# 10XGenomics/supernova

Measured on AMD Instinct MI355X. Metric: Gk-mers/s through count+graph at k=48, 1.2B×150bp; bit-exact counts, higher is better.
Workload: dtype u64

## Files before the change

### include/snk.h

```cpp
#ifndef SNK_H_
#define SNK_H_
#include <stddef.h>
#include <stdint.h>

#ifdef __cplusplus
extern "C" {
#endif

#define SNK_OK 0
#define SNK_E_ARG (-1)
#define SNK_E_HIP (-2)
#define SNK_E_NOGPU (-3)
#define SNK_E_NOMEM (-4)
#define SNK_E_IO (-5)
#define SNK_E_UNSUPPORTED (-6)
#define SNK_E_INTERNAL (-7)

typedef struct snk_ctx snk_ctx;

typedef struct snk_params {
    uint32_t K;
    uint32_t min_qual;
    uint32_t min_freq;
    uint32_t min_bc;
// ... 26 lines not shown
    uint32_t count_tight_slots;
    uint32_t count_screen_ratio_pct;
    uint32_t target_inst;
    uint32_t bucket_fill_pct;
    uint32_t adaptive_buckets;
    uint32_t chunk_kmers;
    uint32_t minimiser_len;
    uint32_t partition_passes;
    uint32_t hot_buckets;
    uint32_t hot_min, hot_factor, hot_class_inst;
    uint32_t exchange_ranges;
    uint32_t join_ranking;
    uint32_t path_lookup;
    uint32_t unitig_bc_cut;
    uint32_t hbv_dev_min, hbv_big;
    uint32_t reserved[9];
    uint32_t last_count_kernel, last_count_limit, last_partition_passes, last_minimiser_len;
} snk_tuning;
void snk_tuning_default(snk_tuning* t);
int snk_ctx_set_tuning(snk_ctx* ctx, const snk_tuning* t, char* err, size_t errcap);
void snk_ctx_get_tuning(const snk_ctx* ctx, snk_tuning* t);
int snk_ctx_set_option(snk_ctx* ctx, const char* name, long long value, char* err, size_t errcap);
int snk_option_check(const char* name, long long value, char* err, size_t errcap);
int snk_ctx_clear_option(snk_ctx* ctx, const char* name);
int snk_ctx_get_option(const snk_ctx* ctx, const char* name, long long* value);
const char* snk_option_name(uint32_t i);
const char* snk_option_doc(uint32_t i);

typedef struct snk_synth_params {
    uint64_t seed;
    uint64_t n_reads;
// ... 398 lines not shown
```

### supernova_amd/csrc/snk_api.hip

```cpp
#include <math.h>
#include <stdlib.h>
#include <execinfo.h>
#include <dlfcn.h>
#include <time.h>

#include <algorithm>

#include "snk_ctx.h"
#include "snk_kernels.h"
#include "snk_synth.h"

static thread_local char g_last_error[512] = "";

hipError_t snk_enter(snk_ctx* ctx) { return hipSetDevice(ctx->device); }

void snk_set_mlen(snk_ctx* ctx, const snk_params* p) {
    uint32_t m = (p->flags & SNK_F_LONG_MINIMISER) ? (uint32_t)SNK_M_LONG : (uint32_t)SNK_M_OF(p->K);
    const unsigned long long v = snk_opt_u64(ctx, SNK_OPT_minimiser_len);
    if (v == SNK_M_LONG || v == SNK_M_OF(p->K)) m = (uint32_t)v;
    ctx->mlen = m;
}

void snk_set_error(char* err, size_t errcap, const char* fmt, ...) {
    va_list ap;
// ... 390 lines not shown
    }
    ctx->blocks.swap(keep);
}

extern "C" void snk_ctx_destroy(snk_ctx* ctx) {
    if (!ctx) return;
    (void)snk_enter(ctx);
    snk_ctx_release_scratch(ctx);
    snk_ctx_trim_cache(ctx);
    if (ctx->va_base) { va_unmap_from(ctx, 0); (void)hipMemAddressFree(ctx->va_base, ctx->va_size); ctx->va_base = nullptr; }
    if (ctx->shard) snk_shard_state_free(ctx->shard);
    if (ctx->host_io && ctx->host_io_free) ctx->host_io_free(ctx->host_io);
    if (ctx->df_io && ctx->df_io_free) ctx->df_io_free(ctx->df_io);
    if (ctx->shard_host && ctx->shard_host_free) ctx->shard_host_free(ctx->shard_host);
    if (ctx->stream_job && ctx->stream_job_free) ctx->stream_job_free(ctx->stream_job);
    if (ctx->stream) (void)hipStreamDestroy(ctx->stream);
    delete ctx;
}

extern "C" void snk_synth_default(snk_synth_params* sp, uint64_t n_reads, uint64_t seed, int error_free) {
    memset(sp, 0, sizeof *sp);
    sp->seed = seed;
    sp->n_reads = n_reads;
    sp->read_len = 150;
    sp->genome_len = n_reads * 150 / 56;
    if (sp->genome_len < 1000) sp->genome_len = 1000;
    sp->mol_len = 50000;
    sp->mols_per_bc = 10;
    sp->pairs_per_bc = 400;
    sp->insert_min = 300;
// ... 53 lines not shown
```

### supernova_amd/csrc/snk_ctx.h

```cpp
#pragma once
#include <hip/hip_runtime.h>
#include <stdarg.h>
#include <stdio.h>
#include <string.h>

#include <string>
#include <vector>

#include "../../include/snk.h"
#include "snk_launch.h"
#include "snk_opts.h"

struct snk_ctx {
    int device = 0;
    hipStream_t stream = nullptr;
    hipStream_t cur_stream = nullptr;
    int n_cu = 256;
    size_t lds_per_block = 65536;
    uint64_t device_mem_total = 0;
    double pass_sigma = 0.0;
    uint64_t plan_mapped = 0;
    uint64_t plan_mem = 0;
    struct block { void* p; size_t bytes; bool used; uint64_t serial = 0; uint64_t epoch = 0; };
    uint64_t call_epoch = 0;
    uint64_t alloc_serial = 0;
    std::vector<block> blocks;
    struct vrange { size_t off, bytes; };
    char* va_base = nullptr;
    size_t va_size = 0, va_mapped = 0, va_high = 0, va_high_prev[2] = {0, 0};
    std::vector<hipMemGenericAllocationHandle_t> va_handles;
    std::vector<size_t> va_chunk;
    std::vector<vrange> va_free;
    std::vector<vrange> va_used;
    size_t va_floor = 0;
    int va_state = 0;
    bool va_sealed = false;
    struct vser { size_t off; uint64_t serial; };
    std::vector<vser> va_serial;
    bool arena_legacy = false;
    size_t total_alloc = 0;
    size_t peak_alloc = 0;
    size_t cached_bytes = 0;
    uint64_t last_n_kmers = 0, last_n_instances = 0;
    uint64_t last_region_max = 0, last_region_n = 0;
    uint64_t last_bnd = 0, last_bnd_n = 0;
    uint32_t last_ovf = 0, last_ovf_nb = 0;
    uint64_t last_ovf_reads = 0;
    uint64_t last_dense = 0;
    double retain_ratio = 0.0;
    uint32_t count_screen = 0;
    uint32_t count_tight = 0;
    double screen_ratio = 0.0;
    double claim_ratio = 0.0;
    uint64_t claim_ratio_reads = 0;
    uint32_t claim_ratio_k = 0;
    uint32_t mlen = 16;
    uint32_t last_extra = 0;
    uint64_t last_input_fp = 0;
    bool have_input_fp = false;
    uint32_t last_count_limit = 0;
// ... 40 lines not shown
```

### supernova_amd/csrc/snk_local.hip

```cpp
#include <string.h>
#include <cstring>
#include <rocprim/rocprim.hpp>

#include <type_traits>

#include "snk_ctx.h"
#include "snk_common.h"
#include "snk_kernels.h"
#include "snk_graph.h"
#include "snk_stages.h"

namespace {

constexpr uint32_t NONE = 0xFFFFFFFFu;
constexpr unsigned long long NONE64 = ~0ull;
constexpr uint16_t NONE16 = 0xFFFFu;
constexpr int TB = 256;

struct chunk_src {
    const uint32_t* chunk_n;
    const uint32_t* chunk_base;
    const uint4* extra;
    const unsigned long long* region_off;
    uint32_t NB, n_extra, n_regions;
// ... 21 lines not shown
    if (r >= G) return;
    uint32_t head = NONE, total = 0, m = 0, expect = 0;
    for (uint32_t b = r; b < NB; b += G) {
        const uint32_t n = chunk_n[b];
        span[b] = 1;
        merged[b] = n;
        if (n == 0) { head = NONE; continue; }
        const uint32_t base = chunk_base[b];
        if (head != NONE && base == expect && total + n <= cap && m < 255u) {
            total += n; ++m;
            merged[head] = total; merged[b] = 0; span[head] = (uint8_t)m;
        } else { head = b; total = n; m = 1; }
        expect = base + n;
    }
}
__global__ void __launch_bounds__(256) bl_chunk_desc_kernel(chunk_src cs, uint32_t nchunks, uint4* __restrict__ desc, uint64_t region_cap, uint64_t* __restrict__ desc_src) {
    const uint32_t c = blockIdx.x * 256 + threadIdx.x;
    if (c >= nchunks) return;
    uint32_t bucket, n, off = 0, meta = 0, region;
    if (c < cs.NB) {
        bucket = c; n = cs.chunk_n[c];
        if (n) off = cs.chunk_base[c];
        region = bucket % cs.n_regions;
        if (cs.span && n && cs.span[c] > 1) meta = 0x80000000u | cs.span[c];
    } else {
        const uint4 e = cs.extra[c - cs.NB];
        bucket = e.x; off = e.y; n = e.z & 0xFFFu; region = e.z >> 12; meta = e.w;
    }
    const uint64_t base = cs.region_off[region] + off;
    desc[c] = make_uint4((uint32_t)base, n, bucket, meta);
    if (desc_src) desc_src[c] = (uint64_t)region * region_cap + off;
}
__device__ __forceinline__ chunk_t chunk_get(const uint4* __restrict__ desc, uint32_t c) {
    const uint4 d = desc[c];
    chunk_t k;
    k.base = d.x; k.n = d.y; k.bucket = d.z; k.lg = d.w >> 24; k.id = d.w & 0xFFFFFFu; k.span = 1;
    if (d.w >> 31) { k.lg = 0; k.id = 0; k.span = d.w & 0xFFFFu; }
    return k;
}

__device__ __forceinline__ snk_kmer load_key(const snk_u128* keys, uint64_t i) {
    const uint64_t* p = reinterpret_cast<const uint64_t*>(keys + i);
    snk_kmer k;
    k.lo = p[0];
    k.hi = p[1];
    return k;
// ... 2 lines not shown
    uint32_t x = (uint32_t)(hi >> 32) * 0x9E3779B1u ^ (uint32_t)hi * 0x85EBCA77u ^ (uint32_t)(lo >> 32) * 0xC2B2AE3Du ^
                 (uint32_t)lo * 0x27D4EB2Fu;
    return snk_mix32(x);
}
template <int K>
__device__ __forceinline__ uint32_t oriented_base(snk_kmer k, bool rc, int idx) {
    return rc ? (snk_kmer_base<K>(k, K - 1 - idx) ^ 3u) : snk_kmer_base<K>(k, idx);
}

template <int K, int CAP, int T, bool BIG, bool GR, int MM>
__device__ __forceinline__ void bl_prune_chunk(const uint32_t c, const uint4* __restrict__ desc, uint32_t NB, bl_shard sh, const bl_regions& rg,
                                                     const snk_u128* __restrict__ keys, const uint64_t* __restrict__ vals,
                                                     uint32_t do_prune, uint8_t* __restrict__ ctx_out,
                                                     uint32_t* __restrict__ count_out, uint8_t* __restrict__ pend_out,
                                                     uint32_t* __restrict__ nbr_out, uint32_t* __restrict__ nbnd,
                                                     uint32_t* __restrict__ biglist, uint32_t* __restrict__ nbig,
                                                     unsigned long long* __restrict__ gindex, uint64_t gmask) {
    constexpr int HT = CAP <= 256 ? 512 : 4096;
    typedef typename std::conditional<(K <= 48 && !GR), uint32_t, uint64_t>::type klo_w;
    constexpr int KLS = (K <= 48 && !GR) ? 32 : 0;
    __shared__ uint64_t khi[CAP];
    __shared__ klo_w klo[CAP];
    __shared__ uint32_t ht[HT];
    __shared__ uint32_t bcnt;
    const int tid = threadIdx.x;
    const chunk_t ch = chunk_get(desc, c);
    if (ch.n == 0) return;
    if (!BIG && ch.n > (uint32_t)CAP) {
        if (tid == 0) biglist[atomicAdd(nbig, 1u)] = c;
        return;
    }
    const uint32_t n = ch.n;
    uint64_t src = ch.base;
    if (rg.keys_r) { src = rg.desc_src[c]; keys = rg.keys_r; vals = rg.vals_r; }
    __syncthreads();
    for (int s = tid; s < HT; s += T) ht[s] = 0;
    if (tid == 0) bcnt = 0;
    constexpr int NPT = (CAP + T - 1) / T;
    uint64_t myv[NPT];
    snk_kmer kq[NPT];
#pragma unroll
    for (int q = 0; q < NPT; ++q) {
        const uint32_t i = tid + q * T;
        myv[q] = 0;
        if (i < n) {
            kq[q] = load_key(keys, src + i);
// ... 156 lines not shown
                    if (!placed) gindex[gmask + 1] = 1ull;
                }
            }
        }
    }
    snk_wave_add(&bcnt, mybnd);
    __syncthreads();
    if (tid == 0) nbnd[c] = bcnt;
}
template <int K, int CAP, int T, bool BIG, bool GR, int MM>
__global__ void __launch_bounds__(T) bl_prune_kernel(const uint4* __restrict__ desc, uint32_t NB, bl_shard sh, bl_regions rg, const uint32_t* __restrict__ biglist_in,
                                                     uint32_t nchunks, uint32_t cpw,
                                                     const snk_u128* __restrict__ keys, const uint64_t* __restrict__ vals,
                                                     uint32_t do_prune, uint8_t* __restrict__ ctx_out,
                                                     uint32_t* __restrict__ count_out, uint8_t* __restrict__ pend_out,
                                                     uint32_t* __restrict__ nbr_out, uint32_t* __restrict__ nbnd,
                                                     uint32_t* __restrict__ biglist, uint32_t* __restrict__ nbig, const uint32_t* __restrict__ n_dev,
                                                     unsigned long long* __restrict__ gindex, uint64_t gmask) {
    if (BIG && n_dev) {
        const uint32_t nb = *n_dev;
        for (uint32_t w = blockIdx.x; w < nb; w += gridDim.x)
            bl_prune_chunk<K, CAP, T, BIG, GR, MM>(biglist_in[w], desc, NB, sh, rg, keys, vals, do_prune, ctx_out, count_out, pend_out, nbr_out, nbnd, biglist, nbig, gindex, gmask);
        return;
    }
    for (uint32_t r = 0; r < cpw; ++r) {
        const uint32_t w = blockIdx.x * cpw + r;
        if (w >= nchunks) return;
        bl_prune_chunk<K, CAP, T, BIG, GR, MM>(BIG ? biglist_in[w] : w, desc, NB, sh, rg, keys, vals, do_prune, ctx_out, count_out, pend_out, nbr_out,
                                       nbnd, biglist, nbig, gindex, gmask);
    }
}

__global__ void __launch_bounds__(TB) bl_index_build_kernel(const snk_u128* __restrict__ keys, const uint8_t* __restrict__ pend,
                                                            uint64_t n, unsigned long long* __restrict__ tab, uint64_t mask) {
    const uint64_t i = (uint64_t)blockIdx.x * TB + threadIdx.x;
    if (i >= n || !pend[i]) return;
    const snk_kmer k = load_key(keys, i);
    uint32_t h1, h2;
    snk_kmer_hash2(k, &h1, &h2);
    uint64_t slot = (((uint64_t)h1 << 32) | h2) & mask;
    const unsigned long long ent = ((unsigned long long)h1 << 32) | (unsigned long long)(i + 1);
    for (;;) {
        const unsigned long long old = atomicCAS(&tab[slot], 0ull, ent);
        if (old == 0ull) break;
// ... 378 lines not shown
template <typename T>
static int excl_scan(snk_ctx* ctx, hipStream_t st, const T* in, T* out, size_t count, char* err, size_t errcap) {
    size_t tb = 0;
    SNK_HIP_TRY(rocprim::exclusive_scan((void*)nullptr, tb, in, out, (T)0, count, rocprim::plus<T>(), st));
    void* tmp;
    int rc = snk_ctx_alloc(ctx, tb, &tmp, err, errcap);
    if (rc) return rc;
    SNK_HIP_TRY(rocprim::exclusive_scan(tmp, tb, in, out, (T)0, count, rocprim::plus<T>(), st));
    return SNK_OK;
}

constexpr int SCAP = 256, ST = 64;
constexpr int BCAP = SNK_GRAPH_CHUNK_MAX, BT = 256;

namespace {
constexpr int QWORDS = 4;
constexpr int QSPAN = 8 * QWORDS * TB;
template <int K, bool FILL>
__global__ void __launch_bounds__(TB) bl_query_kernel(const snk_u128* __restrict__ keys, const uint8_t* __restrict__ premote, uint64_t n,
                                                      uint32_t NB_total, uint32_t NBl, uint32_t world, uint32_t mlen,
                                                      unsigned long long* __restrict__ qcount_or_cursor,
                                                      unsigned long long* __restrict__ qbuf) {
    extern __shared__ unsigned long long dynq[];
    __shared__ uint16_t list[QSPAN];
    __shared__ uint32_t cnt;
    uint32_t* lcur = reinterpret_cast<uint32_t*>(dynq + world);
    const uint64_t base = (uint64_t)blockIdx.x * QSPAN;
    if (threadIdx.x == 0) cnt = 0;
    for (uint32_t r = threadIdx.x; r < world; r += TB) { dynq[r] = 0; lcur[r] = 0; }
    __syncthreads();
// ... 64 lines not shown
    const uint32_t merge_cap = snk_opt_is_set(ctx, SNK_OPT_chunk_merge) ? std::min<uint32_t>(snk_opt_u32(ctx, SNK_OPT_chunk_merge), (uint32_t)SCAP) : (uint32_t)SCAP;
    if (merge_cap && tab->chunk_n && tab->NB > tab->n_regions) {
        uint8_t* span;
        uint32_t* merged;
        G_ALLOC(span, uint8_t, (uint64_t)tab->NB + 1);
        G_ALLOC(merged, uint32_t, (uint64_t)tab->NB + 1);
        SNK_HIP_TRY(snk_launch(bl_chunk_merge_kernel, snk_blocks(tab->n_regions, 256), 256, 0, st, tab->chunk_n, tab->chunk_base, tab->NB, tab->n_regions, merge_cap, span, merged));
        cs.span = span;
        cs.chunk_n = merged;
    }
    const uint32_t nchunks = tab->NB + tab->n_extra;
    B->nchunks = nchunks;
    G_ALLOC(B->desc, uint4, (uint64_t)nchunks + 1);
    uint64_t* desc_src = nullptr;
    if (tab->keys_r) G_ALLOC(desc_src, uint64_t, (uint64_t)nchunks + 1);
    SNK_HIP_TRY(snk_launch(bl_chunk_desc_kernel, snk_blocks(nchunks, 256), 256, 0, st, cs, nchunks, B->desc, tab->region_cap, desc_src));
    uint32_t *nbnd, *ctr;
    G_ALLOC(B->ctx, uint8_t, n + 16);
    G_ALLOC(B->pend, uint8_t, n + 16);
    G_ALLOC(B->counts, uint32_t, n + 4);
    G_ALLOC(B->nbr, uint32_t, n + 2);
    G_ALLOC(B->rq, uint32_t, 2 * n + 2);
    G_ALLOC(nbnd, uint32_t, (uint64_t)nchunks + 1);
    G_ALLOC(B->biglist, uint32_t, n / SCAP + 2);
    G_ALLOC(ctr, uint32_t, 16);
    B->premote = nullptr;
    if (B->world > 1 || B->force_dist) {
        G_ALLOC(B->premote, uint8_t, n + 16);
        SNK_HIP_TRY(hipMemsetAsync(B->premote, 0, n + 16, st));
    }
    SNK_HIP_TRY(hipMemsetAsync(nbnd, 0, ((uint64_t)nchunks + 1) * 4, st));
    SNK_HIP_TRY(hipMemsetAsync(ctr, 0, 64, st));
    bl_shard sh;
    sh.bucket_base = B->premote ? B->rank * B->NBl : 0u;
    sh.NBl = B->premote ? B->NBl : 0u;
    sh.me = B->rank;
    sh.G = tab->n_regions ? tab->n_regions : 1u;
    sh.premote = B->premote;
    const uint32_t NBh = B->premote ? B->NB_total : tab->NB;
    const uint32_t cpw = snk_opt_u32(ctx, SNK_OPT_bl_cpw);
    uint64_t tg0 = 0;
    unsigned long long* index0 = nullptr;
    if (snk_opt_u32(ctx, SNK_OPT_bl_index_fused)) {
        const uint64_t guess = (ctx->last_bnd_n == n && ctx->last_bnd) ? ctx->last_bnd + ctx->last_bnd / 8 : n / 5;
        tg0 = 1024;
        while (tg0 < 2 * guess) tg0 <<= 1;
        G_ALLOC(index0, unsigned long long, tg0 + 1);
        SNK_HIP_TRY(hipMemsetAsync(index0, 0, (tg0 + 1) * 8, st));
    }
    bl_regions rg;
    rg.keys_r = tab->keys_r; rg.vals_r = tab->vals_r; rg.desc_src = desc_src;
    rg.keys_dense = const_cast<snk_u128*>(tab->keys);
    const bool long_m = ctx->mlen == (uint32_t)SNK_M_LONG;
    SNK_HIP_TRY(snk_launch(long_m ? bl_prune_kernel<K, SCAP, ST, false, GR, SNK_M_LONG> : bl_prune_kernel<K, SCAP, ST, false, GR, SNK_M_OF(K)>, snk_blocks(nchunks, cpw), ST, 0, st, (const uint4*)B->desc, NBh, sh, rg,
                           (const uint32_t*)nullptr, nchunks, cpw, tab->keys, tab->vals, B->do_prune | (snk_opt_u32(ctx, SNK_OPT_bl_noclassify) ? 2u : 0u), B->ctx, B->counts, B->pend, B->nbr, nbnd,
                           B->biglist, ctr, (const uint32_t*)nullptr, index0, tg0 - 1));
    uint32_t h_nbig = 0;
    SNK_HIP_TRY(hipMemcpyAsync(ctr + 1, ctr, 4, hipMemcpyDeviceToDevice, st));
    SNK_HIP_TRY(snk_launch(long_m ? bl_prune_kernel<K, BCAP, BT, true, GR, SNK_M_LONG> : bl_prune_kernel<K, BCAP, BT, true, GR, SNK_M_OF(K)>, 2048, BT, 0, st, (const uint4*)B->desc, NBh, sh, rg,
                           (const uint32_t*)B->biglist, 0u, 1u, tab->keys, tab->vals, B->do_prune | (snk_opt_u32(ctx, SNK_OPT_bl_noclassify) ? 2u : 0u), B->ctx, B->counts, B->pend, B->nbr,
                           nbnd, B->biglist, ctr + 2, (const uint32_t*)(ctr + 1), index0, tg0 - 1));
    if (tab->keys_r) {
        snk_ctx_release_block(ctx, tab->keys_r);
        snk_ctx_release_block(ctx, tab->vals_r);
    }
    unsigned long long* d_sum;
    G_ALLOC(d_sum, unsigned long long, 2);
    {
        size_t tb = 0;
        auto in = rocprim::make_transform_iterator(nbnd, [] __device__(uint32_t v) { return (unsigned long long)v; });
        SNK_HIP_TRY(rocprim::reduce((void*)nullptr, tb, in, d_sum, 0ull, (size_t)nchunks, rocprim::plus<unsigned long long>(), st));
        void* tmp;
        int rc = snk_ctx_alloc(ctx, tb, &tmp, err, errcap);
        if (rc) return rc;
        SNK_HIP_TRY(rocprim::reduce(tmp, tb, in, d_sum, 0ull, (size_t)nchunks, rocprim::plus<unsigned long long>(), st));
    }
    unsigned long long h_bnd = 0, h_gaveup = 0;
    if (index0) SNK_HIP_TRY(hipMemcpyAsync(&h_gaveup, index0 + tg0, 8, hipMemcpyDeviceToHost, st));
    SNK_HIP_TRY(hipMemcpyAsync(&h_bnd, d_sum, 8, hipMemcpyDeviceToHost, st));
    SNK_HIP_TRY(hipMemcpyAsync(&h_nbig, ctr + 1, 4, hipMemcpyDeviceToHost, st));
    SNK_HIP_TRY(snk_sync(st));
    B->nbig = h_nbig;
    B->n_boundary = h_bnd;
    ctx->last_bnd = h_bnd; ctx->last_bnd_n = n;
    uint64_t tg = 1024;
    while (tg < 2 * h_bnd) tg <<= 1;
    const bool fused_ok = index0 && !h_gaveup && h_bnd * 4 <= tg0 * 3;
    if (fused_ok) { B->index = index0; tg = tg0; }
    else {
        if (index0) snk_ctx_release_block(ctx, index0);
        G_ALLOC(B->index, unsigned long long, tg);
        SNK_HIP_TRY(hipMemsetAsync(B->index, 0, tg * 8, st));
    }
    B->index_mask = tg - 1;
    if (h_bnd) {
        if (!fused_ok) SNK_HIP_TRY(snk_launch(bl_index_build_kernel, snk_blocks(n, TB), TB, 0, st, tab->keys, B->pend, n, B->index, tg - 1));
        SNK_HIP_TRY(snk_launch(bl_resolve_kernel<K, GR>, snk_blocks(n, 8 * TB), TB, 0, st, tab->keys, B->pend, n,
// ... 4 lines not shown

template <int K, bool DIST, bool GR>
static int bl_fragments_impl(snk_ctx* ctx, hipStream_t st, snk_bl_state* B, const bl_dist_args& da, snk_frag_out* out, char* err,
                             size_t errcap) {
    const snk_table* tab = B->tab;
    const uint32_t nchunks = B->nchunks, h_nbig = B->nbig;
    uint32_t *nfrag, *foff;
    uint64_t *nbases, *boff;
    G_ALLOC(nfrag, uint32_t, (uint64_t)nchunks + 1);
    G_ALLOC(foff, uint32_t, (uint64_t)nchunks + 1);
    G_ALLOC(nbases, uint64_t, (uint64_t)nchunks + 1);
    G_ALLOC(boff, uint64_t, (uint64_t)nchunks + 1);
    SNK_HIP_TRY(hipMemsetAsync(nfrag, 0, ((uint64_t)nchunks + 1) * 4, st));
    bl_extra_pool xp0;
    memset(&xp0, 0, sizeof xp0);
    SNK_HIP_TRY(snk_launch(bl_frag_kernel<K, SCAP, ST, false, false, DIST, GR>, nchunks, ST, 0, st, (const uint4*)B->desc,
                           (const uint32_t*)nullptr, tab->keys, B->ctx, B->pend, B->nbr, B->rq, da, nfrag, (const uint32_t*)nullptr,
                           (const uint64_t*)nullptr, (uint32_t*)nullptr, (unsigned long long*)nullptr, (unsigned long long*)nullptr,
                           (uint64_t*)nullptr, (uint8_t*)nullptr, (uint32_t*)nullptr, (uint32_t*)nullptr, xp0));
    SNK_HIP_TRY(snk_launch(bl_frag_kernel<K, BCAP, BT, true, false, DIST, GR>, h_nbig, BT, 0, st, (const uint4*)B->desc,
                           (const uint32_t*)B->biglist, tab->keys, B->ctx, B->pend, B->nbr, B->rq, da, nfrag, (const uint32_t*)nullptr,
                           (const uint64_t*)nullptr, (uint32_t*)nullptr, (unsigned long long*)nullptr, (unsigned long long*)nullptr,
                           (uint64_t*)nullptr, (uint8_t*)nullptr, (uint32_t*)nullptr, (uint32_t*)nullptr, xp0));
    SNK_HIP_TRY(snk_launch(bl_chunk_bases_kernel, snk_blocks((uint64_t)nchunks + 1, TB), TB, 0, st, (const uint4*)B->desc, nfrag, nchunks,
                           (uint32_t)K, nbases));
    int rc;
    if ((rc = excl_scan<uint32_t>(ctx, st, nfrag, foff, (size_t)nchunks + 1, err, errcap))) return rc;
    if ((rc = excl_scan<uint64_t>(ctx, st, nbases, boff, (size_t)nchunks + 1, err, errcap))) return rc;
    uint32_t h_F = 0;
    uint64_t h_B = 0;
    SNK_HIP_TRY(hipMemcpyAsync(&h_F, foff + nchunks, 4, hipMemcpyDeviceToHost, st));
    SNK_HIP_TRY(hipMemcpyAsync(&h_B, boff + nchunks, 8, hipMemcpyDeviceToHost, st));
    SNK_HIP_TRY(snk_sync(st));
    unsigned long long* xcur;
    G_ALLOC(xcur, unsigned long long, 2);
    const uint32_t pool0 = snk_opt_u32(ctx, SNK_OPT_bl_pool);
    uint64_t xf_cap = pool0 ? pool0 + h_F / 256 : 0, xb_cap = xf_cap * (K + 63);
    unsigned long long h_x[2] = {0, 0};
// ... 1 lines not shown
        G_ALLOC(out->nk, uint32_t, (uint64_t)h_F + xf_cap + 1);
        G_ALLOC(out->hl_self, unsigned long long, 2ull * (h_F + xf_cap) + 2);
        G_ALLOC(out->hl_nb, unsigned long long, 2ull * (h_F + xf_cap) + 2);
        G_ALLOC(out->boff, uint64_t, (uint64_t)h_F + xf_cap + 2);
        G_ALLOC(out->bases, uint8_t, h_B + xb_cap + 16);
        out->fgroup = nullptr;
        if (GR) G_ALLOC(out->fgroup, uint32_t, (uint64_t)h_F + xf_cap + 1);
        G_ALLOC(out->sfrag, uint32_t, 2 * tab->n + 2);
        SNK_HIP_TRY(hipMemsetAsync(xcur, 0, 16, st));
        bl_extra_pool xp;
        xp.cur = xcur;
        xp.f0 = h_F;
        xp.b0 = h_B;
        xp.fcap = xf_cap;
        xp.bcap = xb_cap;
        SNK_HIP_TRY(snk_launch(bl_frag_kernel<K, SCAP, ST, false, true, DIST, GR>, nchunks, ST, 0, st, (const uint4*)B->desc,
                               (const uint32_t*)nullptr, tab->keys, B->ctx, B->pend, B->nbr, B->rq, da, nfrag, foff, boff, out->nk, out->hl_self,
                               out->hl_nb, out->boff, out->bases, out->fgroup, out->sfrag, xp));
        SNK_HIP_TRY(snk_launch(bl_frag_kernel<K, BCAP, BT, true, true, DIST, GR>, h_nbig, BT, 0, st, (const uint4*)B->desc,
                               (const uint32_t*)B->biglist, tab->keys, B->ctx, B->pend, B->nbr, B->rq, da, nfrag, foff, boff, out->nk,
                               out->hl_self, out->hl_nb, out->boff, out->bases, out->fgroup, out->sfrag, xp));
        SNK_HIP_TRY(hipMemcpyAsync(h_x, xcur, 16, hipMemcpyDeviceToHost, st));
        SNK_HIP_TRY(snk_sync(st));
        if (h_x[0] <= xf_cap && h_x[1] <= xb_cap) break;
        if (attempt == 1) return snk_fail(SNK_E_INTERNAL, err, errcap, "bucket-local graph: circle pool overflow");
        xf_cap = h_x[0] + 64;
        xb_cap = h_x[1] + 64;
    }
    out->n_frags = h_F + h_x[0];
    out->total_bases = h_B + h_x[1];
    out->n_local_circles = (uint32_t)h_x[0];
    return SNK_OK;
}

template <int K, bool GR>
static int local_graph_impl(snk_ctx* ctx, hipStream_t st, const snk_table* tab, uint32_t do_prune, bool want_unitigs,
// ... 159 lines not shown
```

### supernova_amd/csrc/snk_opts.h

```cpp
#pragma once
#include <stdint.h>

#define SNK_SW 0, 1, 1, false
#define SNK_R(lo, hi) lo, hi, 1, false
#define SNK_R0(lo, hi) lo, hi, 1, true
#define SNK_RS(lo, hi, step) lo, hi, step, false
#define SNK_RS0(lo, hi, step) lo, hi, step, true
#define SNK_U32 4294967295ll

#define SNK_OPTIONS(X) \
     \
     \
    X(count_tight, 0, SNK_R0(256, 1984), "count kernel with booked table slots: 0 never, n = always, n usable slots of the table (256 .. slots - 64); unset: chosen from the data") \
    X(count_screen, 1, SNK_R(0, 2), "per-barcode groups: bit filter in front of the table: 0 off, 1 on for min_freq >= 3 (default), 2 on for min_freq >= 2") \
    X(count_screen_ng, 1, SNK_R(0, 2), "ungrouped reads: bit filter in front of a 1024-slot table: 0 never, 1 when the tables run full (default), 2 always") \
    X(screen_ratio_pct, 30, SNK_R(0, 100), "count_screen_ng = 1: distinct k-mers per 100 instances above which the filter goes on (30)") \
     \
    X(screen_target, 4000, SNK_R(100, 1048576), "k-mer instances per bucket behind the ungrouped filter (4000)") \
     \
    X(tight_tries, 48, SNK_R(1, 65535), "booked slots: how often a wave looks again before it gives the pass up (48)") \
    X(target_inst, 0, SNK_R(100, 1048576), "k-mer instances per minimiser bucket; unset: 5000 (K=48) / 3500 (K=60), adapted to the data") \
    X(bucket_fill_pct, 50, SNK_R(1, 100), "adaptive buckets aim at this share of the table's usable slots (50)") \
    X(adaptive_buckets, 1, SNK_SW, "look at the first buckets of unknown data and partition a second time if their tables run full (1)") \
    X(chunk_kmers, 180, SNK_R(1, 65536), "retained k-mers per bucket the bucket count aims at when the data retain many (180)") \
// ... 10 lines not shown
    X(msp_dense, 0, SNK_SW, "1: reservation-free partition (dense records + sorted index list)") \
    X(msp_hot_factor, 32, SNK_R(0, 65536), "a bucket is noted hot at this multiple of its capacity (32; 0 never)") \
    X(msp_hot_min, 4096, SNK_R(1, SNK_U32), "... and at least this many reservations (4096)") \
    X(trim_fused, 1, SNK_SW, "quality trim inside the partition kernel (1)") \
    X(trim_rowwise, 0, SNK_SW, "1: the row-wise trim kernel for every layout") \
    X(defer_compact, 1, SNK_SW, "leave the count regions in place until the prune reads them (1)") \
     \
    X(hot, 1, SNK_SW, "re-partition hot minimiser buckets by k-mer hash (1)") \
    X(hot_min, 8192, SNK_R(1, SNK_U32), "a bucket is hot above this many records (8192) ...") \
    X(hot_factor, 8, SNK_R(1, 65536), "... and this multiple of the slot capacity (8)") \
    X(hot_class_inst, 6000, SNK_R(100, 1048576), "k-mer instances per hash class of a hot bucket (6000)") \
     \
    X(chunk_merge, 0, SNK_R(0, 65536), "graph chunks are merged up to this many k-mers (256, which is also the most; 0 off)") \
    X(bl_cpw, 4, SNK_R(1, 1024), "graph chunks per workgroup of the prune (4)") \
    X(bl_index_fused, 1, SNK_SW, "boundary index built by the prune (1)") \
    X(bl_noclassify, 0, SNK_SW, "1: every miss of the prune is pending (no neighbour classification)") \
    X(bl_pool, 4096, SNK_R(0, 1048576), "slots of the in-chunk circle pool (4096; 0 forces the exact re-run)") \
     \
    X(split_log2, 5, SNK_R(1, 12), "log2 of the ranking's splitter spacing (5: one state in 32)") \
    X(rank_wyllie, 0, SNK_SW, "1: plain pointer jumping instead of the sparse ruling set") \
    X(emit_grid_log2, 22, SNK_R(0, 22), "log2 of the largest grid of the join's fragment copy (22; tests make it small: the kernel strides)") \
    X(lean_cold, 1, SNK_SW, "0: a context whose arena has not mapped the memory yet still sizes its record slots at 5 sigma (1: 1.5 sigma until the arena has the slack)") \
    X(plan_mem_mb, 0, SNK_R(0, 16777216), "the memory (MB) the slot / pass / region plans of a call divide instead of what the device has free (tests: bucket-range passes and their region probe at fixture size)") \
    X(hbv_huge_pages, 1, SNK_SW, "0: the host tables of a14's flood are plain malloc memory (1: 2-MB aligned with MADV_HUGEPAGE)") \
    X(hbv_short_queue, 1, SNK_SW, "0: the host flood of a14 prefetches 16 / 8 / 4 queue places ahead only (1: also at push time and one / two places ahead: the bulk of a genome graph has a short queue)") \
    X(join_dbg, 0, SNK_SW, "1: the join counts the bytes of its unitig buffers that nothing wrote (stderr; debugging aid)") \
     \
    X(rank_round_batch, 8, SNK_R(1, 64), "jumping rounds per read-back, sharded ranking (8)") \
    X(rank_round_batch0, 12, SNK_R(1, 64), "jumping rounds before the first read-back, one-GPU ranking (12)") \
     \
    X(exchange_ranges, 4, SNK_R(1, 64), "bucket ranges of the record exchange (4; never more than a rank has buckets)") \
// ... 53 lines not shown
```

### supernova_amd/csrc/snk_opts.hip

```cpp
#include <stdio.h>
#include <stdlib.h>
#include <string.h>

#include <string>

#include "snk_ctx.h"
#include "snk_opts.h"

const snk_opt_def snk_opt_defs[SNK_OPT_COUNT] = {
#define X(name, dflt, range, doc) {#name, dflt, range, doc},
    SNK_OPTIONS(X)
#undef X
};

int snk_opt_index(const char* name) {
    if (!name) return -1;
    for (int i = 0; i < SNK_OPT_COUNT; ++i) if (strcmp(snk_opt_defs[i].name, name) == 0) return i;
    return -1;
}
void snk_opts_init(snk_opts* o) { memset(o, 0, sizeof *o); }

int snk_opts_parse(snk_opts* o, const char* text, char* bad, unsigned badcap) {
    if (!text) return 0;
    const char* p = text;
// ... 131 lines not shown
    long long v;
    for (const tfield& f : tfields) if (get(f.opt, &v)) *reinterpret_cast<uint32_t*>(reinterpret_cast<char*>(t) + f.off) = (uint32_t)v;
    long long tight = 0, ng = 0;
    const bool ts = get(SNK_OPT_count_tight, &tight), ns = get(SNK_OPT_count_screen_ng, &ng);
    if (ns && ng >= 2) t->count_kernel = SNK_COUNT_KERNEL_SCREEN;
    else if (ts && tight) { t->count_kernel = SNK_COUNT_KERNEL_BOOKED; t->count_tight_slots = (uint32_t)tight; }
    else if (ts) t->count_kernel = SNK_COUNT_KERNEL_MARGIN;
    if (get(SNK_OPT_adaptive_buckets, &v)) t->adaptive_buckets = v ? 1 : 2;
    if (get(SNK_OPT_hot, &v)) t->hot_buckets = v ? 1 : 2;
    if (get(SNK_OPT_path_index, &v)) t->path_lookup = v ? 1 : 2;
    if (get(SNK_OPT_join_replicated, &v)) t->join_ranking = v ? 2 : 1;
    t->last_count_limit = ctx->last_count_limit;
    t->last_count_kernel = ctx->count_screen ? SNK_COUNT_KERNEL_SCREEN : (ctx->count_tight ? SNK_COUNT_KERNEL_BOOKED : SNK_COUNT_KERNEL_MARGIN);
    t->last_partition_passes = ctx->last_partition_passes;
    t->last_minimiser_len = ctx->mlen;
}
```

### supernova_amd/lib.py

```python
from __future__ import annotations

import ctypes as C
from pathlib import Path

import os as _os

_HERE = Path(__file__).resolve().parent
LIB_PATH = Path(_os.environ.get("SNK_LIB_PATH", str(_HERE / "libsnk.so")))


class SnkError(RuntimeError):
    def __init__(self, code: int, msg: str):
        super().__init__(f"libsnk error {code}: {msg}")
        self.code = code


class SnkParams(C.Structure):
    _fields_ = [("K", C.c_uint32), ("min_qual", C.c_uint32), ("min_freq", C.c_uint32), ("min_bc", C.c_uint32),
                ("n_buckets", C.c_uint32), ("flags", C.c_uint32)]


class SnkSynthParams(C.Structure):
    _fields_ = [("seed", C.c_uint64), ("n_reads", C.c_uint64), ("genome_len", C.c_uint64), ("read_len", C.c_uint32),
                ("mol_len", C.c_uint32), ("mols_per_bc", C.c_uint32), ("pairs_per_bc", C.c_uint32),
# ... 67 lines not shown
                ("text_bytes", C.c_uint64), ("token", C.c_uint64)]


class SnkDevIngest(C.Structure):
    _fields_ = [("n_reads", C.c_uint64), ("read_len", C.c_uint32), ("row_words", C.c_uint32), ("qstride", C.c_uint32),
                ("max_len", C.c_uint32), ("rows", C.c_void_p), ("quals", C.c_void_p), ("lens", C.c_void_p), ("bc", C.c_void_p),
                ("text_bytes", C.c_uint64), ("compressed_bytes", C.c_uint64), ("seconds", C.c_double),
                ("decode_wait_seconds", C.c_double), ("n_files", C.c_uint32), ("n_batches", C.c_uint32), ("setup_seconds", C.c_double), ("good_len", C.c_void_p)]


class SnkTuning(C.Structure):
    _fields_ = [("count_kernel", C.c_uint32), ("count_tight_slots", C.c_uint32), ("count_screen_ratio_pct", C.c_uint32), ("target_inst", C.c_uint32),
                ("bucket_fill_pct", C.c_uint32), ("adaptive_buckets", C.c_uint32), ("chunk_kmers", C.c_uint32), ("minimiser_len", C.c_uint32),
                ("partition_passes", C.c_uint32), ("hot_buckets", C.c_uint32), ("hot_min", C.c_uint32), ("hot_factor", C.c_uint32),
                ("hot_class_inst", C.c_uint32), ("exchange_ranges", C.c_uint32), ("join_ranking", C.c_uint32), ("path_lookup", C.c_uint32),
                ("unitig_bc_cut", C.c_uint32), ("hbv_dev_min", C.c_uint32), ("hbv_big", C.c_uint32), ("reserved", C.c_uint32 * 9),
                ("last_count_kernel", C.c_uint32), ("last_count_limit", C.c_uint32), ("last_partition_passes", C.c_uint32),
                ("last_minimiser_len", C.c_uint32)]


class SnkDfInfo(C.Structure):
    _fields_ = [("n_reads", C.c_uint64), ("n_barcodes", C.c_uint64), ("fastb_bytes", C.c_uint64), ("qualp_bytes", C.c_uint64),
                ("bci_bytes", C.c_uint64), ("reserved", C.c_uint64 * 3)]


class SnkShardResult(C.Structure):
    _fields_ = [("rank", C.c_uint32), ("world", C.c_uint32), ("n_reads", C.c_uint64), ("n_instances", C.c_uint64),
                ("n_supermers", C.c_uint64), ("n_buckets_total", C.c_uint64), ("n_kmers", C.c_uint64), ("keys", C.c_void_p),
                ("counts", C.c_void_p), ("ctx", C.c_void_p), ("spectrum", C.c_void_p), ("spectrum_bins", C.c_uint32),
                ("n_circles", C.c_uint32), ("n_unitigs", C.c_uint64), ("unitig_total_bases", C.c_uint64),
                ("unitig_off", C.c_void_p), ("unitig_bases", C.c_void_p), ("unitig_circular", C.c_void_p),
                ("n_frags", C.c_uint64), ("n_frags_total", C.c_uint64), ("n_queries", C.c_uint64), ("n_link_queries", C.c_uint64),
# ... 192 lines not shown
```

Before: 97.65.

## Classify big graph chunks up front and run big-chunk kernels on a side stream

The chunk descriptor kernel now builds the list of oversized chunks, so the small-chunk prune kernel no longer has to discover and append them. This lets the big-chunk prune, size and emit kernels launch on a second non-blocking stream, forked and joined with events, concurrently with the small-chunk kernels instead of serialised after them. The fork is skipped when the previous run of the same size had no big chunks, and option bit 2 restores single-stream ordering. The cost is event and stream bookkeeping, plus the two kernel sets competing for CUs and memory bandwidth.

```diff
diff --git a/include/snk.h b/include/snk.h
--- a/include/snk.h
+++ b/include/snk.h
@@ -64,7 +64,8 @@
     uint32_t path_lookup;
     uint32_t unitig_bc_cut;
     uint32_t hbv_dev_min, hbv_big;
-    uint32_t reserved[9];
+    uint32_t reserved[8];
+    uint32_t last_big_chunks;
     uint32_t last_count_kernel, last_count_limit, last_partition_passes, last_minimiser_len;
 } snk_tuning;
 void snk_tuning_default(snk_tuning* t);
diff --git a/supernova_amd/csrc/snk_api.hip b/supernova_amd/csrc/snk_api.hip
--- a/supernova_amd/csrc/snk_api.hip
+++ b/supernova_amd/csrc/snk_api.hip
@@ -428,6 +428,9 @@
     if (ctx->df_io && ctx->df_io_free) ctx->df_io_free(ctx->df_io);
     if (ctx->shard_host && ctx->shard_host_free) ctx->shard_host_free(ctx->shard_host);
     if (ctx->stream_job && ctx->stream_job_free) ctx->stream_job_free(ctx->stream_job);
+    if (ctx->side_fork) (void)hipEventDestroy(ctx->side_fork);
+    if (ctx->side_join) (void)hipEventDestroy(ctx->side_join);
+    if (ctx->side_stream) (void)hipStreamDestroy(ctx->side_stream);
     if (ctx->stream) (void)hipStreamDestroy(ctx->stream);
     delete ctx;
 }
diff --git a/supernova_amd/csrc/snk_ctx.h b/supernova_amd/csrc/snk_ctx.h
--- a/supernova_amd/csrc/snk_ctx.h
+++ b/supernova_amd/csrc/snk_ctx.h
@@ -15,6 +15,8 @@
     int device = 0;
     hipStream_t stream = nullptr;
     hipStream_t cur_stream = nullptr;
+    hipStream_t side_stream = nullptr;
+    hipEvent_t side_fork = nullptr, side_join = nullptr;
     int n_cu = 256;
     size_t lds_per_block = 65536;
     uint64_t device_mem_total = 0;
@@ -44,6 +46,7 @@
     uint64_t last_n_kmers = 0, last_n_instances = 0;
     uint64_t last_region_max = 0, last_region_n = 0;
     uint64_t last_bnd = 0, last_bnd_n = 0;
+    uint32_t last_nbig = 0; uint64_t last_nbig_n = ~0ull;
     uint32_t last_ovf = 0, last_ovf_nb = 0;
     uint64_t last_ovf_reads = 0;
     uint64_t last_dense = 0;
diff --git a/supernova_amd/csrc/snk_local.hip b/supernova_amd/csrc/snk_local.hip
--- a/supernova_amd/csrc/snk_local.hip
+++ b/supernova_amd/csrc/snk_local.hip
@@ -59,7 +59,8 @@
         expect = base + n;
     }
 }
-__global__ void __launch_bounds__(256) bl_chunk_desc_kernel(chunk_src cs, uint32_t nchunks, uint4* __restrict__ desc, uint64_t region_cap, uint64_t* __restrict__ desc_src) {
+__global__ void __launch_bounds__(256) bl_chunk_desc_kernel(chunk_src cs, uint32_t nchunks, uint4* __restrict__ desc, uint64_t region_cap, uint64_t* __restrict__ desc_src,
+                                                            uint32_t small_cap, uint32_t* __restrict__ biglist, uint32_t* __restrict__ nbig) {
     const uint32_t c = blockIdx.x * 256 + threadIdx.x;
     if (c >= nchunks) return;
     uint32_t bucket, n, off = 0, meta = 0, region;
@@ -75,6 +76,7 @@
     const uint64_t base = cs.region_off[region] + off;
     desc[c] = make_uint4((uint32_t)base, n, bucket, meta);
     if (desc_src) desc_src[c] = (uint64_t)region * region_cap + off;
+    if (n > small_cap) biglist[atomicAdd(nbig, 1u)] = c;
 }
 __device__ __forceinline__ chunk_t chunk_get(const uint4* __restrict__ desc, uint32_t c) {
     const uint4 d = desc[c];
@@ -107,7 +109,6 @@
                                                      uint32_t do_prune, uint8_t* __restrict__ ctx_out,
                                                      uint32_t* __restrict__ count_out, uint8_t* __restrict__ pend_out,
                                                      uint32_t* __restrict__ nbr_out, uint32_t* __restrict__ nbnd,
-                                                     uint32_t* __restrict__ biglist, uint32_t* __restrict__ nbig,
                                                      unsigned long long* __restrict__ gindex, uint64_t gmask) {
     constexpr int HT = CAP <= 256 ? 512 : 4096;
     typedef typename std::conditional<(K <= 48 && !GR), uint32_t, uint64_t>::type klo_w;
@@ -119,10 +120,7 @@
     const int tid = threadIdx.x;
     const chunk_t ch = chunk_get(desc, c);
     if (ch.n == 0) return;
-    if (!BIG && ch.n > (uint32_t)CAP) {
-        if (tid == 0) biglist[atomicAdd(nbig, 1u)] = c;
-        return;
-    }
+    if (!BIG && ch.n > (uint32_t)CAP) return;
     const uint32_t n = ch.n;
     uint64_t src = ch.base;
     if (rg.keys_r) { src = rg.desc_src[c]; keys = rg.keys_r; vals = rg.vals_r; }
@@ -309,20 +307,19 @@
                                                      const snk_u128* __restrict__ keys, const uint64_t* __restrict__ vals,
                                                      uint32_t do_prune, uint8_t* __restrict__ ctx_out,
                                                      uint32_t* __restrict__ count_out, uint8_t* __restrict__ pend_out,
-                                                     uint32_t* __restrict__ nbr_out, uint32_t* __restrict__ nbnd,
-                                                     uint32_t* __restrict__ biglist, uint32_t* __restrict__ nbig, const uint32_t* __restrict__ n_dev,
+                                                     uint32_t* __restrict__ nbr_out, uint32_t* __restrict__ nbnd, const uint32_t* __restrict__ n_dev,
                                                      unsigned long long* __restrict__ gindex, uint64_t gmask) {
     if (BIG && n_dev) {
         const uint32_t nb = *n_dev;
         for (uint32_t w = blockIdx.x; w < nb; w += gridDim.x)
-            bl_prune_chunk<K, CAP, T, BIG, GR, MM>(biglist_in[w], desc, NB, sh, rg, keys, vals, do_prune, ctx_out, count_out, pend_out, nbr_out, nbnd, biglist, nbig, gindex, gmask);
+            bl_prune_chunk<K, CAP, T, BIG, GR, MM>(biglist_in[w], desc, NB, sh, rg, keys, vals, do_prune, ctx_out, count_out, pend_out, nbr_out, nbnd, gindex, gmask);
         return;
     }
     for (uint32_t r = 0; r < cpw; ++r) {
         const uint32_t w = blockIdx.x * cpw + r;
         if (w >= nchunks) return;
         bl_prune_chunk<K, CAP, T, BIG, GR, MM>(BIG ? biglist_in[w] : w, desc, NB, sh, rg, keys, vals, do_prune, ctx_out, count_out, pend_out, nbr_out,
-                                       nbnd, biglist, nbig, gindex, gmask);
+                                       nbnd, gindex, gmask);
     }
 }
 
@@ -731,6 +728,38 @@
 constexpr int BCAP = SNK_GRAPH_CHUNK_MAX, BT = 256;
 
 namespace {
+struct bl_side {
+    snk_ctx* ctx;
+    hipStream_t st;
+    bool on, open = false;
+    bl_side(snk_ctx* c, hipStream_t s, bool want) : ctx(c), st(s), on(want) {}
+    ~bl_side() { if (open) (void)join(); }
+    hipStream_t side() const { return on ? ctx->side_stream : st; }
+    hipError_t fork() {
+        if (!on) return hipSuccess;
+        hipError_t e;
+        if (!ctx->side_stream) {
+            if ((e = hipStreamCreateWithFlags(&ctx->side_stream, hipStreamNonBlocking)) != hipSuccess) return e;
+            if ((e = hipEventCreateWithFlags(&ctx->side_fork, hipEventDisableTiming)) != hipSuccess) return e;
+            if ((e = hipEventCreateWithFlags(&ctx->side_join, hipEventDisableTiming)) != hipSuccess) return e;
+        }
+        if ((e = hipEventRecord(ctx->side_fork, st)) != hipSuccess) return e;
+        if ((e = hipStreamWaitEvent(ctx->side_stream, ctx->side_fork, 0)) != hipSuccess) return e;
+        open = true;
+        return hipSuccess;
+    }
+    hipError_t join() {
+        if (!open) return hipSuccess;
+        open = false;
+        hipError_t e;
+        if ((e = hipEventRecord(ctx->side_join, ctx->side_stream)) != hipSuccess) return e;
+        return hipStreamWaitEvent(st, ctx->side_join, 0);
+    }
+};
+bool bl_overlap_wanted(const snk_ctx* ctx) { return !(snk_opt_u32(ctx, SNK_OPT_bl_noclassify) & 2u); }
+}
+
+namespace {
 constexpr int QWORDS = 4;
 constexpr int QSPAN = 8 * QWORDS * TB;
 template <int K, bool FILL>
@@ -825,23 +854,23 @@
     G_ALLOC(B->desc, uint4, (uint64_t)nchunks + 1);
     uint64_t* desc_src = nullptr;
     if (tab->keys_r) G_ALLOC(desc_src, uint64_t, (uint64_t)nchunks + 1);
-    SNK_HIP_TRY(snk_launch(bl_chunk_desc_kernel, snk_blocks(nchunks, 256), 256, 0, st, cs, nchunks, B->desc, tab->region_cap, desc_src));
     uint32_t *nbnd, *ctr;
+    G_ALLOC(B->biglist, uint32_t, n / SCAP + 2);
+    G_ALLOC(ctr, uint32_t, 16);
+    SNK_HIP_TRY(hipMemsetAsync(ctr, 0, 64, st));
+    SNK_HIP_TRY(snk_launch(bl_chunk_desc_kernel, snk_blocks(nchunks, 256), 256, 0, st, cs, nchunks, B->desc, tab->region_cap, desc_src, (uint32_t)SCAP, B->biglist, ctr));
     G_ALLOC(B->ctx, uint8_t, n + 16);
     G_ALLOC(B->pend, uint8_t, n + 16);
     G_ALLOC(B->counts, uint32_t, n + 4);
     G_ALLOC(B->nbr, uint32_t, n + 2);
     G_ALLOC(B->rq, uint32_t, 2 * n + 2);
     G_ALLOC(nbnd, uint32_t, (uint64_t)nchunks + 1);
-    G_ALLOC(B->biglist, uint32_t, n / SCAP + 2);
-    G_ALLOC(ctr, uint32_t, 16);
     B->premote = nullptr;
     if (B->world > 1 || B->force_dist) {
         G_ALLOC(B->premote, uint8_t, n + 16);
         SNK_HIP_TRY(hipMemsetAsync(B->premote, 0, n + 16, st));
     }
     SNK_HIP_TRY(hipMemsetAsync(nbnd, 0, ((uint64_t)nchunks + 1) * 4, st));
-    SNK_HIP_TRY(hipMemsetAsync(ctr, 0, 64, st));
     bl_shard sh;
     sh.bucket_base = B->premote ? B->rank * B->NBl : 0u;
     sh.NBl = B->premote ? B->NBl : 0u;
@@ -863,14 +892,20 @@
     rg.keys_r = tab->keys_r; rg.vals_r = tab->vals_r; rg.desc_src = desc_src;
     rg.keys_dense = const_cast<snk_u128*>(tab->keys);
     const bool long_m = ctx->mlen == (uint32_t)SNK_M_LONG;
+    const uint32_t prune_mode = B->do_prune | ((snk_opt_u32(ctx, SNK_OPT_bl_noclassify) & 1u) ? 2u : 0u);
+    bl_side fk(ctx, st, bl_overlap_wanted(ctx) && !(ctx->last_nbig_n == n && ctx->last_nbig == 0));
+    auto prune_big = [&](hipStream_t s) {
+        return snk_launch(long_m ? bl_prune_kernel<K, BCAP, BT, true, GR, SNK_M_LONG> : bl_prune_kernel<K, BCAP, BT, true, GR, SNK_M_OF(K)>, 2048, BT, 0, s, (const uint4*)B->desc, NBh, sh, rg,
+                          (const uint32_t*)B->biglist, 0u, 1u, tab->keys, tab->vals, prune_mode, B->ctx, B->counts, B->pend, B->nbr, nbnd, (const uint32_t*)ctr, index0, tg0 - 1);
+    };
+    SNK_HIP_TRY(fk.fork());
+    if (fk.on) SNK_HIP_TRY(prune_big(fk.side()));
     SNK_HIP_TRY(snk_launch(long_m ? bl_prune_kernel<K, SCAP, ST, false, GR, SNK_M_LONG> : bl_prune_kernel<K, SCAP, ST, false, GR, SNK_M_OF(K)>, snk_blocks(nchunks, cpw), ST, 0, st, (const uint4*)B->desc, NBh, sh, rg,
-                           (const uint32_t*)nullptr, nchunks, cpw, tab->keys, tab->vals, B->do_prune | (snk_opt_u32(ctx, SNK_OPT_bl_noclassify) ? 2u : 0u), B->ctx, B->counts, B->pend, B->nbr, nbnd,
-                           B->biglist, ctr, (const uint32_t*)nullptr, index0, tg0 - 1));
+                           (const uint32_t*)nullptr, nchunks, cpw, tab->keys, tab->vals, prune_mode, B->ctx, B->counts, B->pend, B->nbr, nbnd,
+                           (const uint32_t*)nullptr, index0, tg0 - 1));
+    if (!fk.on) SNK_HIP_TRY(prune_big(st));
+    SNK_HIP_TRY(fk.join());
     uint32_t h_nbig = 0;
-    SNK_HIP_TRY(hipMemcpyAsync(ctr + 1, ctr, 4, hipMemcpyDeviceToDevice, st));
-    SNK_HIP_TRY(snk_launch(long_m ? bl_prune_kernel<K, BCAP, BT, true, GR, SNK_M_LONG> : bl_prune_kernel<K, BCAP, BT, true, GR, SNK_M_OF(K)>, 2048, BT, 0, st, (const uint4*)B->desc, NBh, sh, rg,
-                           (const uint32_t*)B->biglist, 0u, 1u, tab->keys, tab->vals, B->do_prune | (snk_opt_u32(ctx, SNK_OPT_bl_noclassify) ? 2u : 0u), B->ctx, B->counts, B->pend, B->nbr,
-                           nbnd, B->biglist, ctr + 2, (const uint32_t*)(ctr + 1), index0, tg0 - 1));
     if (tab->keys_r) {
         snk_ctx_release_block(ctx, tab->keys_r);
         snk_ctx_release_block(ctx, tab->vals_r);
@@ -889,9 +924,10 @@
     unsigned long long h_bnd = 0, h_gaveup = 0;
     if (index0) SNK_HIP_TRY(hipMemcpyAsync(&h_gaveup, index0 + tg0, 8, hipMemcpyDeviceToHost, st));
     SNK_HIP_TRY(hipMemcpyAsync(&h_bnd, d_sum, 8, hipMemcpyDeviceToHost, st));
-    SNK_HIP_TRY(hipMemcpyAsync(&h_nbig, ctr + 1, 4, hipMemcpyDeviceToHost, st));
+    SNK_HIP_TRY(hipMemcpyAsync(&h_nbig, ctr, 4, hipMemcpyDeviceToHost, st));
     SNK_HIP_TRY(snk_sync(st));
     B->nbig = h_nbig;
+    ctx->last_nbig = h_nbig; ctx->last_nbig_n = n;
     B->n_boundary = h_bnd;
     ctx->last_bnd = h_bnd; ctx->last_bnd_n = n;
     uint64_t tg = 1024;
@@ -926,14 +962,21 @@
     SNK_HIP_TRY(hipMemsetAsync(nfrag, 0, ((uint64_t)nchunks + 1) * 4, st));
     bl_extra_pool xp0;
     memset(&xp0, 0, sizeof xp0);
+    bl_side fk(ctx, st, bl_overlap_wanted(ctx) && h_nbig > 0);
+    auto size_big = [&](hipStream_t s) {
+        return snk_launch(bl_frag_kernel<K, BCAP, BT, true, false, DIST, GR>, h_nbig, BT, 0, s, (const uint4*)B->desc,
+                          (const uint32_t*)B->biglist, tab->keys, B->ctx, B->pend, B->nbr, B->rq, da, nfrag, (const uint32_t*)nullptr,
+                          (const uint64_t*)nullptr, (uint32_t*)nullptr, (unsigned long long*)nullptr, (unsigned long long*)nullptr,
+                          (uint64_t*)nullptr, (uint8_t*)nullptr, (uint32_t*)nullptr, (uint32_t*)nullptr, xp0);
+    };
+    SNK_HIP_TRY(fk.fork());
+    if (fk.on) SNK_HIP_TRY(size_big(fk.side()));
     SNK_HIP_TRY(snk_launch(bl_frag_kernel<K, SCAP, ST, false, false, DIST, GR>, nchunks, ST, 0, st, (const uint4*)B->desc,
                            (const uint32_t*)nullptr, tab->keys, B->ctx, B->pend, B->nbr, B->rq, da, nfrag, (const uint32_t*)nullptr,
                            (const uint64_t*)nullptr, (uint32_t*)nullptr, (unsigned long long*)nullptr, (unsigned long long*)nullptr,
                            (uint64_t*)nullptr, (uint8_t*)nullptr, (uint32_t*)nullptr, (uint32_t*)nullptr, xp0));
-    SNK_HIP_TRY(snk_launch(bl_frag_kernel<K, BCAP, BT, true, false, DIST, GR>, h_nbig, BT, 0, st, (const uint4*)B->desc,
-                           (const uint32_t*)B->biglist, tab->keys, B->ctx, B->pend, B->nbr, B->rq, da, nfrag, (const uint32_t*)nullptr,
-                           (const uint64_t*)nullptr, (uint32_t*)nullptr, (unsigned long long*)nullptr, (unsigned long long*)nullptr,
-                           (uint64_t*)nullptr, (uint8_t*)nullptr, (uint32_t*)nullptr, (uint32_t*)nullptr, xp0));
+    if (!fk.on) SNK_HIP_TRY(size_big(st));
+    SNK_HIP_TRY(fk.join());
     SNK_HIP_TRY(snk_launch(bl_chunk_bases_kernel, snk_blocks((uint64_t)nchunks + 1, TB), TB, 0, st, (const uint4*)B->desc, nfrag, nchunks,
                            (uint32_t)K, nbases));
     int rc;
@@ -965,12 +1008,18 @@
         xp.b0 = h_B;
         xp.fcap = xf_cap;
         xp.bcap = xb_cap;
+        auto emit_big = [&](hipStream_t s) {
+            return snk_launch(bl_frag_kernel<K, BCAP, BT, true, true, DIST, GR>, h_nbig, BT, 0, s, (const uint4*)B->desc,
+                              (const uint32_t*)B->biglist, tab->keys, B->ctx, B->pend, B->nbr, B->rq, da, nfrag, foff, boff, out->nk,
+                              out->hl_self, out->hl_nb, out->boff, out->bases, out->fgroup, out->sfrag, xp);
+        };
+        SNK_HIP_TRY(fk.fork());
+        if (fk.on) SNK_HIP_TRY(emit_big(fk.side()));
         SNK_HIP_TRY(snk_launch(bl_frag_kernel<K, SCAP, ST, false, true, DIST, GR>, nchunks, ST, 0, st, (const uint4*)B->desc,
                                (const uint32_t*)nullptr, tab->keys, B->ctx, B->pend, B->nbr, B->rq, da, nfrag, foff, boff, out->nk, out->hl_self,
                                out->hl_nb, out->boff, out->bases, out->fgroup, out->sfrag, xp));
-        SNK_HIP_TRY(snk_launch(bl_frag_kernel<K, BCAP, BT, true, true, DIST, GR>, h_nbig, BT, 0, st, (const uint4*)B->desc,
-                               (const uint32_t*)B->biglist, tab->keys, B->ctx, B->pend, B->nbr, B->rq, da, nfrag, foff, boff, out->nk,
-                               out->hl_self, out->hl_nb, out->boff, out->bases, out->fgroup, out->sfrag, xp));
+        if (!fk.on) SNK_HIP_TRY(emit_big(st));
+        SNK_HIP_TRY(fk.join());
         SNK_HIP_TRY(hipMemcpyAsync(h_x, xcur, 16, hipMemcpyDeviceToHost, st));
         SNK_HIP_TRY(snk_sync(st));
         if (h_x[0] <= xf_cap && h_x[1] <= xb_cap) break;
diff --git a/supernova_amd/csrc/snk_opts.h b/supernova_amd/csrc/snk_opts.h
--- a/supernova_amd/csrc/snk_opts.h
+++ b/supernova_amd/csrc/snk_opts.h
@@ -48,7 +48,8 @@
     X(chunk_merge, 0, SNK_R(0, 65536), "graph chunks are merged up to this many k-mers (256, which is also the most; 0 off)") \
     X(bl_cpw, 4, SNK_R(1, 1024), "graph chunks per workgroup of the prune (4)") \
     X(bl_index_fused, 1, SNK_SW, "boundary index built by the prune (1)") \
-    X(bl_noclassify, 0, SNK_SW, "1: every miss of the prune is pending (no neighbour classification)") \
+     \
+    X(bl_noclassify, 0, SNK_R(0, 3), "1: every miss of the prune is pending (no neighbour classification); 2: the big-chunk launches behind the one-wave ones on one stream instead of next to them; 3: both") \
     X(bl_pool, 4096, SNK_R(0, 1048576), "slots of the in-chunk circle pool (4096; 0 forces the exact re-run)") \
      \
     X(split_log2, 5, SNK_R(1, 12), "log2 of the ranking's splitter spacing (5: one state in 32)") \
diff --git a/supernova_amd/csrc/snk_opts.hip b/supernova_amd/csrc/snk_opts.hip
--- a/supernova_amd/csrc/snk_opts.hip
+++ b/supernova_amd/csrc/snk_opts.hip
@@ -169,4 +169,5 @@
     t->last_count_kernel = ctx->count_screen ? SNK_COUNT_KERNEL_SCREEN : (ctx->count_tight ? SNK_COUNT_KERNEL_BOOKED : SNK_COUNT_KERNEL_MARGIN);
     t->last_partition_passes = ctx->last_partition_passes;
     t->last_minimiser_len = ctx->mlen;
+    t->last_big_chunks = ctx->last_nbig;
 }
diff --git a/supernova_amd/lib.py b/supernova_amd/lib.py
--- a/supernova_amd/lib.py
+++ b/supernova_amd/lib.py
@@ -105,8 +105,8 @@
                 ("bucket_fill_pct", C.c_uint32), ("adaptive_buckets", C.c_uint32), ("chunk_kmers", C.c_uint32), ("minimiser_len", C.c_uint32),
                 ("partition_passes", C.c_uint32), ("hot_buckets", C.c_uint32), ("hot_min", C.c_uint32), ("hot_factor", C.c_uint32),
                 ("hot_class_inst", C.c_uint32), ("exchange_ranges", C.c_uint32), ("join_ranking", C.c_uint32), ("path_lookup", C.c_uint32),
-                ("unitig_bc_cut", C.c_uint32), ("hbv_dev_min", C.c_uint32), ("hbv_big", C.c_uint32), ("reserved", C.c_uint32 * 9),
-                ("last_count_kernel", C.c_uint32), ("last_count_limit", C.c_uint32), ("last_partition_passes", C.c_uint32),
+                ("unitig_bc_cut", C.c_uint32), ("hbv_dev_min", C.c_uint32), ("hbv_big", C.c_uint32), ("reserved", C.c_uint32 * 8),
+                ("last_big_chunks", C.c_uint32), ("last_count_kernel", C.c_uint32), ("last_count_limit", C.c_uint32), ("last_partition_passes", C.c_uint32),
                 ("last_minimiser_len", C.c_uint32)]
 
 
```

Result: no change. 97.57 (-0.1%).
